# huangjh-pub/di-fusion

Hardware: AMD Instinct MI355X
Metric: frames/s integrate+decode+mesh, 640x480 synthetic stream (higher is better)
Workload: dtype f32

## Files before the change

### di_fusion_amd/csrc/kernels_extract.hip.h

```cpp
#pragma once

__device__ __forceinline__ void mark_confident_nbhd(const Geo& g, int lin, float ignore_th, const int64_t* __restrict__ indexer,
                                                    const float* __restrict__ obs, const GridMarks& marks) {
    const uint32_t* bits = marks.bits;
    int ix, iy, iz;
    unlinearize(g, lin, ix, iy, iz);
    int cand[7];
    cand[0] = lin;
    cand[1] = linearize(g, clampi(ix - 1, 0, g.nx - 1), iy, iz);
    cand[2] = linearize(g, clampi(ix + 1, 0, g.nx - 1), iy, iz);
    cand[3] = linearize(g, ix, clampi(iy - 1, 0, g.ny - 1), iz);
    cand[4] = linearize(g, ix, clampi(iy + 1, 0, g.ny - 1), iz);
    cand[5] = linearize(g, ix, iy, clampi(iz - 1, 0, g.nz - 1));
    cand[6] = linearize(g, ix, iy, clampi(iz + 1, 0, g.nz - 1));
    int64_t slot[7];
#pragma unroll
    for (int c = 0; c < 7; ++c) slot[c] = indexer[cand[c]];
    float w[7];
#pragma unroll
    for (int c = 0; c < 7; ++c) w[c] = slot[c] >= 0 ? obs[slot[c]] : ignore_th;
    uint32_t word[7];
#pragma unroll
    for (int c = 0; c < 7; ++c) word[c] = (w[c] > ignore_th) ? bits[cand[c] >> 5] : 0xFFFFFFFFu;
    uint32_t prev[7];
// ... 265 lines not shown
        if (R.live) {
            const int64_t p = A.list[row];
            float xn, yn, zn; int ix, iy, iz;
            voxel_of(A.geo, A.xyz[p * 3 + 0], A.xyz[p * 3 + 1], A.xyz[p * 3 + 2], xn, yn, zn, ix, iy, iz);
            R.px = (xn - (float)ix) - 0.5f; R.py = (yn - (float)iy) - 0.5f; R.pz = (zn - (float)iz) - 0.5f;
            lat_row = A.latent + A.indexer[linearize(A.geo, ix, iy, iz)] * L;
            R.out_idx = row;
        }
    }
#pragma unroll
    for (int t = 0; t < 16; ++t) {
        const int k = 2 * t + half;
        float v = 0.0f;
        if (R.live) {
            if (row32) v = row32[k];
            else if (k < L) v = lat_row[k];
            else v = (k == L) ? R.px : ((k == L + 1) ? R.py : R.pz);
        }
        xin[t] = v;
    }
    if constexpr (!DENSE) {
        if (A.mode == 2) {
            unsigned nf = 0;
#pragma unroll
            for (int t = 0; t < 16; ++t) nf |= ((__float_as_uint(xin[t]) & 0x7f800000u) == 0x7f800000u) ? 1u : 0u;
            nf |= (unsigned)__shfl_xor((int)nf, 32);
            R.bad = nf != 0;
        }
    }
    return R;
}

template <bool GRAD, bool DENSE = false>
__global__ void __launch_bounds__(GRAD ? 256 : 512, GRAD ? 1 : 2) k_decode(DecodeArgs A, const float* __restrict__ wblob) {
    extern __shared__ __attribute__((aligned(16))) float lds[];
    if (DENSE && A.zero_word && blockIdx.x == 0 && threadIdx.x == 0) *A.zero_word = 0;
    stage_weights(lds, wblob, DEC_LDS_FLOATS);
    const __amdgpu_buffer_rsrc_t wfwd = make_rsrc(wblob, DEC_FLOATS);
    const __amdgpu_buffer_rsrc_t wbwd = make_rsrc(GRAD ? A.wbwd : wblob, GRAD ? DECB_FLOATS : DEC_FLOATS);
    const int lane = lane_id(), half = lane >> 5, col = lane & 31;
    const int wave = (int)((threadIdx.x >> 6) * gridDim.x + blockIdx.x);
    const int nwaves = (int)(gridDim.x * (blockDim.x >> 6));
    const int res3 = A.lat.res * A.lat.res * A.lat.res;
    const int tiles_per_voxel = (res3 + 31) / 32;
    int64_t n_rows, n_tiles;
    if (A.mode == 0) {
        n_rows = (int64_t)(*A.n_ptr) * res3;
        n_tiles = (int64_t)(*A.n_ptr) * tiles_per_voxel;
    } else {
        n_rows = A.n_ptr ? (int64_t)(*A.n_ptr) : A.n_static;
        n_tiles = (n_rows + 31) / 32;
    }
    for (int64_t tile = wave; tile < n_tiles; tile += nwaves) {
        f16v xin;
        const DecodeRow R = decode_row_input<DENSE>(A, tile, col, half, res3, tiles_per_voxel, n_rows, xin);
        const bool live = R.live;
        const int64_t out_idx = R.out_idx;
        const float px = R.px, py = R.py, pz = R.pz;
        float sdf, sd;
        if (!GRAD && A.mode == 1 && A.fold_table) {
            const int b = live ? A.list[tile * 32 + col] / res3 : 0;
            decoder_tile_folded(lds, wfwd, FoldInitGlobal{A.fold_table + (int64_t)b * 256}, px, py, pz, lane, sdf, sd);
        } else if (GRAD) {
            float gx, gy, gz;
            decoder_tile_grad(lds, wfwd, wbwd, xin, lane, sdf, sd, gx, gy, gz);
            if (live && half == 1) {
                const float gs = R.bad ? __builtin_nanf("") : A.grad_scale;
                A.out_grad[out_idx * 3 + 0] = gx * gs;
                A.out_grad[out_idx * 3 + 1] = gy * gs;
                A.out_grad[out_idx * 3 + 2] = gz * gs;
            }
        } else {
            decoder_tile(lds, wfwd, xin, lane, sdf, sd);
        }
        if (live) {
            if (half == 0) A.out_sdf[out_idx] = R.bad ? __builtin_nanf("") : A.sign * sdf;
            else A.out_std[out_idx] = R.bad ? __builtin_nanf("") : sd;
        }
    }
}

template <bool DENSE = false>
__global__ void __launch_bounds__(512, 1) k_decode_x6(DecodeArgs A, const float* __restrict__ wblob, const float* __restrict__ wu) {
    extern __shared__ __attribute__((aligned(16))) float lds[];
    if (DENSE && A.zero_word && blockIdx.x == 0 && threadIdx.x == 0) *A.zero_word = 0;
    stage_weights(lds, wblob, X6_LDS_BYTES / 4);
    const __amdgpu_buffer_rsrc_t wfwd = make_rsrc(wblob, X6_BYTES / 4);
    const __amdgpu_buffer_rsrc_t wun = make_rsrc(wu, X6U_BYTES / 4);
    const int lane = lane_id(), half = lane >> 5, col = lane & 31;
    const int wave = (int)((threadIdx.x >> 6) * gridDim.x + blockIdx.x);
    const int nwaves = (int)(gridDim.x * (blockDim.x >> 6));
    const int res3 = A.lat.res * A.lat.res * A.lat.res;
    const int tiles_per_voxel = (res3 + 31) / 32;
    int64_t n_rows, n_tiles;
    if (A.mode == 0) {
        n_rows = (int64_t)(*A.n_ptr) * res3;
        n_tiles = (int64_t)(*A.n_ptr) * tiles_per_voxel;
    } else {
        n_rows = A.n_ptr ? (int64_t)(*A.n_ptr) : A.n_static;
        n_tiles = (n_rows + 31) / 32;
    }
    for (int64_t tile = wave; tile < n_tiles; tile += nwaves) {
        f16v xin;
        const DecodeRow R = decode_row_input<DENSE>(A, tile, col, half, res3, tiles_per_voxel, n_rows, xin);
        const bool live = R.live;
        const int64_t out_idx = R.out_idx;
        float sdf, sd;
        decoder_tile_x6(lds, wfwd, wun, xin, lane, sdf, sd);
        if (live) {
            if (half == 0) A.out_sdf[out_idx] = R.bad ? __builtin_nanf("") : A.sign * sdf;
            else A.out_std[out_idx] = R.bad ? __builtin_nanf("") : sd;
        }
    }
}

#ifndef GRAD_X6_THREADS
#define GRAD_X6_THREADS 256
#endif
template <int PF, bool DENSE = false>
__global__ void __launch_bounds__(GRAD_X6_THREADS, 1) k_decode_grad_x6(DecodeArgs A, const float* __restrict__ wblob, const float* __restrict__ wu,
                                                          const float* __restrict__ wb) {
    extern __shared__ __attribute__((aligned(16))) float lds[];
    if (DENSE && A.zero_word && blockIdx.x == 0 && threadIdx.x == 0) *A.zero_word = 0;
    stage_weights(lds, wblob, X6_LDS_BYTES / 4);
    const __amdgpu_buffer_rsrc_t wfwd = make_rsrc(wblob, X6_BYTES / 4);
    const __amdgpu_buffer_rsrc_t wun = make_rsrc(wu, X6U_BYTES / 4);
    const __amdgpu_buffer_rsrc_t wbw = make_rsrc(wb, X6B_BYTES / 4);
    const int lane = lane_id(), half = lane >> 5, col = lane & 31;
    const int wave = (int)((threadIdx.x >> 6) * gridDim.x + blockIdx.x);
    const int nwaves = (int)(gridDim.x * (blockDim.x >> 6));
    const int res3 = A.lat.res * A.lat.res * A.lat.res;
    const int64_t n_rows = A.n_ptr ? (int64_t)(*A.n_ptr) : A.n_static;
    const int64_t n_tiles = (n_rows + 31) / 32;
    for (int64_t tile = wave; tile < n_tiles; tile += nwaves) {
        f16v xin;
        const DecodeRow R = decode_row_input<DENSE>(A, tile, col, half, res3, 1, n_rows, xin);
        float sdf, sd, gx, gy, gz;
        decoder_tile_grad_x6<PF>(lds, wfwd, wun, wbw, xin, lane, sdf, sd, gx, gy, gz);
        if (R.live) {
            if (half == 0) A.out_sdf[R.out_idx] = R.bad ? __builtin_nanf("") : A.sign * sdf;
            else {
                const float gs = R.bad ? __builtin_nanf("") : A.grad_scale;
                A.out_std[R.out_idx] = R.bad ? __builtin_nanf("") : sd;
                A.out_grad[R.out_idx * 3 + 0] = gx * gs;
                A.out_grad[R.out_idx * 3 + 1] = gy * gs;
                A.out_grad[R.out_idx * 3 + 2] = gz * gs;
            }
        }
    }
}

template <int NS>
__device__ __forceinline__ void decode_refine_x6_body(const BatchN<DecodeArgs, NS>& B, int S, const float* __restrict__ wblob) {
    extern __shared__ __attribute__((aligned(16))) float lds[];
    const int lane = lane_id(), half = lane >> 5, col = lane & 31;
    const int wave = __builtin_amdgcn_readfirstlane((int)((threadIdx.x >> 6) * gridDim.x + blockIdx.x));
    const int nwaves = (int)(gridDim.x * (blockDim.x >> 6));
    const Lattice lat = B.s[0].lat;
    const float sign = B.s[0].sign;
    const int res3 = lat.res * lat.res * lat.res, r = lat.res;
    Ranges<NS, int64_t> rg;
    rg.pre[0] = 0;
#pragma unroll
    for (int j = 0; j < NS; ++j) {
        rg.cnt[j] = (j < S) ? (B.s[j].n_ptr ? (int64_t)(*B.s[j].n_ptr) : B.s[j].n_static) : 0;
        rg.pre[j + 1] = rg.pre[j] + (rg.cnt[j] + 31) / 32;
    }
    const int64_t n_tiles = rg.total();
    int sm_n; int64_t lt_n, rows_n;
    rg.locate(wave, sm_n, lt_n, rows_n);
    int e_next = (wave < n_tiles && lt_n * 32 + col < rows_n) ? B.s[sm_n].list[lt_n * 32 + col] : 0;
    __builtin_amdgcn_sched_barrier(0);
    stage_weights(lds, wblob, X6_LDS_BYTES / 4);
    const __amdgpu_buffer_rsrc_t wfwd = make_rsrc(wblob, X6_BYTES / 4);
    for (int64_t T = wave; T < n_tiles; T += nwaves) {
        const int sm = sm_n;
        const int64_t tile = lt_n, n_rows = rows_n;
        const DecodeArgs& A = B.s[sm];
        const int64_t row = tile * 32 + col;
        const bool live = row < n_rows;
        const int e = e_next;
        rg.locate(T + nwaves, sm_n, lt_n, rows_n);
        e_next = (T + nwaves < n_tiles && lt_n * 32 + col < rows_n) ? B.s[sm_n].list[lt_n * 32 + col] : 0;
        const int b = e / res3, sb = e - b * res3;
        const float px = lat.coord(sb / (r * r)), py = lat.coord((sb / r) % r), pz = lat.coord(sb % r);
        float sdf, sd;
        decoder_tile_folded_x6(lds, wfwd, FoldInitGlobal{A.fold_table + (int64_t)b * 256}, px, py, pz, lane, sdf, sd);
        if (live) {
            if (half == 0) A.out_sdf[e] = sign * sdf;
            else A.out_std[e] = sd;
        }
    }
}

__global__ void __launch_bounds__(512, 1) k_decode_refine_x6(DecodeArgs A, const float* __restrict__ wblob) {
    const BatchN<DecodeArgs, 1> B{{A}};
    decode_refine_x6_body<1>(B, 1, wblob);
}
__global__ void __launch_bounds__(512, 1) k_decode_refine_x6_batch(Batch<DecodeArgs> B, int S, const float* __restrict__ wblob) {
    decode_refine_x6_body<DIF_MAX_STREAMS>(B, S, wblob);
}

__device__ __forceinline__ void tri_axis(int j, int l, float scale, int& i0, int& i1, float& w0, float& w1) {
    float src = scale * (float)j;
    i0 = min((int)src, l - 1);
    i1 = i0 + ((i0 < l - 1) ? 1 : 0);
    w1 = fminf(fmaxf(src - (float)i0, 0.0f), 1.0f);
    w0 = 1.0f - w1;
}

__device__ __forceinline__ float tri_sample(const float* __restrict__ low, int l, int x0, int x1, int y0, int y1, int z0, int z1,
                                            float wx0, float wx1, float wy0, float wy1, float wz0, float wz1) {
    float v00 = fmaf(low[(x0 * l + y0) * l + z0], wz0, low[(x0 * l + y0) * l + z1] * wz1);
    float v01 = fmaf(low[(x0 * l + y1) * l + z0], wz0, low[(x0 * l + y1) * l + z1] * wz1);
    float v10 = fmaf(low[(x1 * l + y0) * l + z0], wz0, low[(x1 * l + y0) * l + z1] * wz1);
    float v11 = fmaf(low[(x1 * l + y1) * l + z0], wz0, low[(x1 * l + y1) * l + z1] * wz1);
    float v0 = fmaf(v00, wy0, v01 * wy1);
    float v1 = fmaf(v10, wy0, v11 * wy1);
    return fmaf(v0, wx0, v1 * wx1);
}

__global__ void __launch_bounds__(DIF_BLOCK) k_upsample_mark(const float* __restrict__ low_sdf, const float* __restrict__ low_std, int l, int R,
                                                           float* __restrict__ cube_sdf, float* __restrict__ cube_std,
                                                           int32_t* __restrict__ refine_list, int* __restrict__ counters) {
    __shared__ int smem[8];
    __shared__ int s_base;
    const int B = counters[DIF_C_B];
    const int R2 = R * R, R3 = R2 * R, l3 = l * l * l;
    const int64_t n_rows = (int64_t)B * R2;
    const float scale = (float)(l - 1) / (float)(R - 1);
    const int64_t stride = (int64_t)gridDim.x * blockDim.x;
    const int64_t n_pad = (n_rows + DIF_BLOCK - 1) / DIF_BLOCK * DIF_BLOCK;
    for (int64_t row = (int64_t)blockIdx.x * blockDim.x + threadIdx.x; row < n_pad; row += stride) {
        unsigned sel = 0;
        int64_t e0 = 0;
        if (row < n_rows) {
            const int b = (int)(row / R2), jxy = (int)(row - (int64_t)b * R2);
            const int jx = jxy / R, jy = jxy % R;
            int x0, x1, y0, y1; float wx0, wx1, wy0, wy1;
            tri_axis(jx, l, scale, x0, x1, wx0, wx1);
            tri_axis(jy, l, scale, y0, y1, wy0, wy1);
            const float* ls = low_sdf + (int64_t)b * l3;
            const float* ld = low_std + (int64_t)b * l3;
            e0 = (int64_t)b * R3 + (int64_t)jxy * R;
            NO_PACKED_F32
            for (int jz = 0; jz < R; ++jz) {
                int z0, z1; float wz0, wz1;
                tri_axis(jz, l, scale, z0, z1, wz0, wz1);
                float sv = tri_sample(ls, l, x0, x1, y0, y1, z0, z1, wx0, wx1, wy0, wy1, wz0, wz1);
                float dv = tri_sample(ld, l, x0, x1, y0, y1, z0, z1, wx0, wx1, wy0, wy1, wz0, wz1);
                cube_sdf[e0 + jz] = -sv;
                cube_std[e0 + jz] = dv;
                if (fabsf(sv) < 0.05f) sel |= 1u << jz;
            }
        }
        int total;
        int ex = block_excl_scan(__popc(sel), smem, total);
        if (total > 0) {
            if (threadIdx.x == 0) s_base = atomicAdd(counters + DIF_C_VH, total);
            __syncthreads();
            int o = s_base + ex;
            while (sel) {
                int jz = __ffs((int)sel) - 1;
                sel &= sel - 1;
                refine_list[o++] = (int32_t)(e0 + jz);
            }
        }
        __syncthreads();
    }
}

struct VoxelDecodeArgs {
    const int32_t* occ_slot;
    const float* latent;
    Lattice low;
    int R;
    float* cube_sdf;
    float* cube_std;
    int32_t* refine_list;
    int* counters;
    const float* fold_w;
    float* fold_table;
};

#define VD_MAX_L3 64
#define VD_MAX_R2 64
#define VD_WAVE_LDS_FLOATS (2 * VD_MAX_L3 + 2 * 256)

#ifdef DIF_TRACE
__device__ unsigned long long g_vd_trace[2048 * 8];
#define VD_STAMP(slot) do { if (lane_id() == 0) g_vd_trace[((threadIdx.x >> 6) * gridDim.x + blockIdx.x) * 8 + (slot)] = wall_clock64(); } while (0)
#else
#define VD_STAMP(slot) do { } while (0)
#endif

template <bool X6, int NS>
__device__ __forceinline__ void decode_voxels_body(const BatchN<VoxelDecodeArgs, NS>& AB, int S, const float* __restrict__ wblob) {
    extern __shared__ __attribute__((aligned(16))) float lds[];
    VD_STAMP(0);
    constexpr int LDS_W = X6 ? X6_LDS_BYTES / 4 : ((DEC_LDS_FLOATS + 3) & ~3);
#if defined(DIF_VD_CUT) && DIF_VD_CUT == 0
    return;
#endif
    stage_weights(lds, wblob, X6 ? X6_LDS_BYTES / 4 : DEC_LDS_FLOATS);
    VD_STAMP(1);
#if defined(DIF_VD_CUT) && DIF_VD_CUT == 1
    return;
#endif
    const __amdgpu_buffer_rsrc_t wfwd = make_rsrc(wblob, X6 ? X6_BYTES / 4 : DEC_FLOATS);
    const int lane = lane_id(), half = lane >> 5, col = lane & 31, wid = threadIdx.x >> 6;
    const int pair = wid >> 1, tsel = wid & 1;
    float* w_low_sdf = lds + LDS_W + pair * VD_WAVE_LDS_FLOATS;
    float* w_low_std = w_low_sdf + VD_MAX_L3;
    float* w_fold = w_low_std + VD_MAX_L3 + tsel * 256;
    const Lattice low = AB.s[0].low;
    const float* const fold_w = AB.s[0].fold_w;
    const int l = low.res, R = AB.s[0].R, l3 = l * l * l, R2 = R * R, R3 = R2 * R;
    const float scale = (float)(l - 1) / (float)(R - 1);
    int pre[NS + 1];
    pre[0] = 0;
#pragma unroll
    for (int j = 0; j < NS; ++j) pre[j + 1] = pre[j] + ((j < S) ? AB.s[j].counters[DIF_C_B] : 0);
    const int B = pre[NS];
    const int pairs_per_block = (int)(blockDim.x >> 7), n_pairs = (int)gridDim.x * pairs_per_block;
    const int first = __builtin_amdgcn_readfirstlane(pair * (int)gridDim.x + (int)blockIdx.x);
    __shared__ int s_tot[8], s_map[8], s_base[NS];
    const int rounds = (B + n_pairs - 1) / n_pairs;
    for (int round = 0; round < rounds; ++round) {
        const int bg = first + round * n_pairs;
        int sm = 0, b = bg;
#pragma unroll
        for (int j = 1; j < NS; ++j)
            if (bg >= pre[j]) { sm = j; b = bg - pre[j]; }
        const VoxelDecodeArgs& A = AB.s[sm];
        unsigned sel = 0;
        const int jz0 = tsel * (R >> 1), jz1 = jz0 + (R >> 1);
        const int64_t e0 = (int64_t)b * R3 + (int64_t)lane * R;
        if (bg < B && tsel * 32 < l3) {
            const float* lat_row = A.latent + (int64_t)A.occ_slot[b] * L;
            const int s = tsel * 32 + col;
            const float px = low.coord(s / (l * l)), py = low.coord((s / l) % l), pz = low.coord(s % l);
            float sdf = 0.0f, sd = 0.0f;
            if (X6 || fold_w) {
                if constexpr (X6) decoder_fold_consts_x6(lds, fold_w, lat_row, w_fold, lane);
                else decoder_fold_consts(lds, fold_w, lat_row, w_fold, lane);
                __builtin_amdgcn_wave_barrier();
                __builtin_amdgcn_s_waitcnt(0xc07f);
                if (tsel == 0) {
                    float* rec = A.fold_table + (int64_t)b * 256;
                    for (int p = lane; p < 256; p += 64) rec[p] = w_fold[p];
                }
                VD_STAMP(6);
#if defined(DIF_VD_CUT) && DIF_VD_CUT == 2
                sdf = w_fold[lane]; sd = w_fold[lane + 64];
#else
                if constexpr (X6) decoder_tile_folded_x6(lds, wfwd, FoldInitLds{w_fold}, px, py, pz, lane, sdf, sd);
                else decoder_tile_folded(lds, wfwd, FoldInitLds{w_fold}, px, py, pz, lane, sdf, sd);
#endif
            } else if constexpr (!X6) {
                f16v xin;
#pragma unroll
                for (int t = 0; t < 16; ++t) {
                    const int k = 2 * t + half;
                    xin[t] = (k < L) ? lat_row[k] : 0.0f;
                }
                if (half) { xin[14] = px; xin[15] = pz; } else { xin[15] = py; }
                decoder_tile(lds, wfwd, xin, lane, sdf, sd);
            }
            if (s < l3) {
                if (half == 0) w_low_sdf[s] = sdf;
                else w_low_std[s] = sd;
            }
        }
        __syncthreads();
        VD_STAMP(2);
        if (bg < B && lane < R2) {
            const int jx = lane / R, jy = lane % R;
            int x0, x1, y0, y1; float wx0, wx1, wy0, wy1;
            tri_axis(jx, l, scale, x0, x1, wx0, wx1);
            tri_axis(jy, l, scale, y0, y1, wy0, wy1);
            float* const cube_sdf = A.cube_sdf;
            float* const cube_std = A.cube_std;
            for (int jz = jz0; jz < jz1; ++jz) {
                int z0, z1; float wz0, wz1;
                tri_axis(jz, l, scale, z0, z1, wz0, wz1);
                float sv = tri_sample(w_low_sdf, l, x0, x1, y0, y1, z0, z1, wx0, wx1, wy0, wy1, wz0, wz1);
                float dv = tri_sample(w_low_std, l, x0, x1, y0, y1, z0, z1, wx0, wx1, wy0, wy1, wz0, wz1);
                cube_sdf[e0 + jz] = -sv;
                cube_std[e0 + jz] = dv;
                if (fabsf(sv) < 0.05f) sel |= 1u << jz;
            }
        }
        VD_STAMP(3);
        const int c = __popc(sel);
        const int incl = wave_incl_scan(c);
        const int total = __shfl(incl, 63);
        if (lane == 0) { s_tot[wid] = total; if (NS > 1) s_map[wid] = sm; }
        __syncthreads();
        if (NS == 1) {
            if (threadIdx.x == 0) {
                int sum = 0;
                for (int w = 0; w < (int)(blockDim.x >> 6); ++w) sum += s_tot[w];
                s_base[0] = sum ? atomicAdd(A.counters + DIF_C_VH, sum) : 0;
            }
        } else if ((int)threadIdx.x < S) {
            const int j = (int)threadIdx.x;
            int sum = 0;
            for (int w = 0; w < (int)(blockDim.x >> 6); ++w) sum += (s_map[w] == j) ? s_tot[w] : 0;
            s_base[j] = sum ? atomicAdd(AB.s[j].counters + DIF_C_VH, sum) : 0;
        }
        __syncthreads();
        if (total > 0) {
            int o = s_base[NS == 1 ? 0 : sm] + incl - c;
            for (int w = 0; w < wid; ++w) o += (NS == 1 || s_map[w] == sm) ? s_tot[w] : 0;
            int32_t* const refine_list = A.refine_list;
            while (sel) {
                const int jz = __ffs((int)sel) - 1;
                sel &= sel - 1;
                refine_list[o++] = (int32_t)(e0 + jz);
            }
        }
        __syncthreads();
        VD_STAMP(4);
    }
    VD_STAMP(5);
}

template <bool X6>
__global__ void __launch_bounds__(512, X6 ? 1 : 2) k_decode_voxels(VoxelDecodeArgs A, const float* __restrict__ wblob) {
    const BatchN<VoxelDecodeArgs, 1> B{{A}};
    decode_voxels_body<X6, 1>(B, 1, wblob);
}
template <bool X6>
__global__ void __launch_bounds__(512, X6 ? 1 : 2) k_decode_voxels_batch(Batch<VoxelDecodeArgs> B, int S, const float* __restrict__ wblob) {
    decode_voxels_body<X6, DIF_MAX_STREAMS>(B, S, wblob);
}
```

### di_fusion_amd/csrc/mlp.hip.h

```cpp
#pragma once
#include "common.hip.h"

namespace dif {

typedef float f16v __attribute__((ext_vector_type(16)));
typedef float f4v __attribute__((ext_vector_type(4)));

__device__ __forceinline__ f16v mfma32(float a, float b, f16v c) { return __builtin_amdgcn_mfma_f32_32x32x2f32(a, b, c, 0, 0, 0); }

__device__ __forceinline__ f16v load_bias16(const float* b, int half) {
    const f4v* p = reinterpret_cast<const f4v*>(b + half * 16);
    f4v b0 = p[0], b1 = p[1], b2 = p[2], b3 = p[3];
    f16v r;
    r[0] = b0.x; r[1] = b0.y; r[2] = b0.z; r[3] = b0.w;
    r[4] = b1.x; r[5] = b1.y; r[6] = b1.z; r[7] = b1.w;
    r[8] = b2.x; r[9] = b2.y; r[10] = b2.z; r[11] = b2.w;
    r[12] = b3.x; r[13] = b3.y; r[14] = b3.z; r[15] = b3.w;
    return r;
}

__device__ __forceinline__ float relu1(float x) { return __int_as_float(max(__float_as_int(x), 0)); }
__device__ __forceinline__ f16v relu16(f16v v) {
#pragma unroll
    for (int i = 0; i < 16; ++i) v[i] = relu1(v[i]);
    return v;
}

typedef unsigned int u4v __attribute__((ext_vector_type(4)));

struct LdsA {
    const f4v* p;
    __device__ __forceinline__ f4v load(int t, int lane) const { return p[t * 64 + lane]; }
};

struct BufA {
    __amdgpu_buffer_rsrc_t rsrc;
    int base;
    __device__ __forceinline__ f4v load(int t, int lane) const {
        u4v v = __builtin_amdgcn_raw_buffer_load_b128(rsrc, lane * 16, base + t * 1024, 0);
        return __builtin_bit_cast(f4v, v);
    }
};

__device__ __forceinline__ __amdgpu_buffer_rsrc_t make_rsrc(const float* p, int n_floats) {
    return __builtin_amdgcn_make_buffer_rsrc((void*)p, 0, n_floats * 4, 0x00020000);
}

template <int NB, class ASRC>
__device__ __forceinline__ f16v block_mm_src(const ASRC& A, const f16v (&hin)[NB], f16v acc, int lane) {
    f4v a = A.load(0, lane);
#pragma unroll
    for (int kb = 0; kb < NB; ++kb) {
#pragma unroll
        for (int g = 0; g < 4; ++g) {
            const int t = kb * 4 + g;
            f4v an = a;
            if (t + 1 < NB * 4) an = A.load(t + 1, lane);
            acc = mfma32(a.x, hin[kb][4 * g + 0], acc);
            acc = mfma32(a.y, hin[kb][4 * g + 1], acc);
            acc = mfma32(a.z, hin[kb][4 * g + 2], acc);
            acc = mfma32(a.w, hin[kb][4 * g + 3], acc);
            a = an;
            __builtin_amdgcn_sched_barrier(0);
        }
    }
    return acc;
}

template <int NMB, int NB, int PF>
__device__ __forceinline__ void stream_mm(const BufA& A, const f16v (&hin)[NB], f16v (&acc)[NMB], int lane) {
    constexpr int NU = NMB * NB * 4;
    f4v ring[PF];
#pragma unroll
    for (int i = 0; i < PF; ++i)
        if (i < NU) ring[i] = A.load(i, lane);
#pragma unroll
    for (int mb = 0; mb < NMB; ++mb) {
#pragma unroll
        for (int kb = 0; kb < NB; ++kb) {
#pragma unroll
            for (int g = 0; g < 4; ++g) {
                const int u = (mb * NB + kb) * 4 + g;
                const f4v a = ring[u % PF];
                if (u + PF < NU) ring[u % PF] = A.load(u + PF, lane);
                acc[mb] = mfma32(a.x, hin[kb][4 * g + 0], acc[mb]);
                acc[mb] = mfma32(a.y, hin[kb][4 * g + 1], acc[mb]);
                acc[mb] = mfma32(a.z, hin[kb][4 * g + 2], acc[mb]);
                acc[mb] = mfma32(a.w, hin[kb][4 * g + 3], acc[mb]);
                __builtin_amdgcn_sched_barrier(0);
            }
        }
    }
}

template <int NB>
__device__ __forceinline__ f16v block_mm(const f4v* __restrict__ A, const f16v (&hin)[NB], f16v acc, int lane) {
    return block_mm_src<NB>(LdsA{A}, hin, acc, lane);
}

#define ENC_A0 0
#define ENC_B0 256
#define ENC_A1 288
#define ENC_B1 2336
#define ENC_A2 2400
#define ENC_B2 18784
#define ENC_A3 19040
#define ENC_B3 27232
#define ENC_FLOATS 27264

__device__ __forceinline__ f16v encoder_tile(const float* __restrict__ W , float x0, float x1, float x2, int lane) {
    const int half = lane >> 5;
    f16v h0[1];
    {
        f16v acc = load_bias16(W + ENC_B0, half);
        f4v a = reinterpret_cast<const f4v*>(W + ENC_A0)[lane];
        acc = mfma32(a.x, x0, acc);
        acc = mfma32(a.y, x1, acc);
        acc = mfma32(a.z, x2, acc);
        h0[0] = relu16(acc);
    }
    f16v h1[2];
#pragma unroll
    for (int mb = 0; mb < 2; ++mb) {
        f16v acc = load_bias16(W + ENC_B1 + mb * 32, half);
        acc = block_mm<1>(reinterpret_cast<const f4v*>(W + ENC_A1) + (mb * 4) * 64, h0, acc, lane);
        h1[mb] = relu16(acc);
    }
    f16v out = load_bias16(W + ENC_B3, half);
#pragma unroll
    for (int mb = 0; mb < 8; ++mb) {
        f16v acc = load_bias16(W + ENC_B2 + mb * 32, half);
        acc = block_mm<2>(reinterpret_cast<const f4v*>(W + ENC_A2) + (mb * 8) * 64, h1, acc, lane);
        f16v h2[1];
        h2[0] = relu16(acc);
        out = block_mm<1>(reinterpret_cast<const f4v*>(W + ENC_A3) + (mb * 4) * 64, h2, out, lane);
    }
    return out;
}

#define DEC_A0 0
#define DEC_B0 4096
#define DEC_A1 4224
#define DEC_B1 20608
#define DEC_A2 20736
#define DEC_B2 33024
#define DEC_B3 33120
#define DEC_HW 33248
#define DEC_HU 33376
#define DEC_HB 33504
#define DEC_LDS_FLOATS 33508
#define DEC_A3 33508
#define DEC_FLOATS 49892

__device__ __forceinline__ void decoder_tile(const float* __restrict__ W , __amdgpu_buffer_rsrc_t Wg ,
                                             const f16v& xin, int lane, float& sdf, float& stdv) {
    const int half = lane >> 5;
    f16v hx[1];
    hx[0] = xin;
    f16v h0[4];
#pragma unroll
    for (int mb = 0; mb < 4; ++mb) {
        f16v acc = load_bias16(W + DEC_B0 + mb * 32, half);
        acc = block_mm<1>(reinterpret_cast<const f4v*>(W + DEC_A0) + (mb * 4) * 64, hx, acc, lane);
        h0[mb] = relu16(acc);
    }
    f16v h1[4];
#pragma unroll
    for (int mb = 0; mb < 4; ++mb) {
        f16v acc = load_bias16(W + DEC_B1 + mb * 32, half);
        acc = block_mm<4>(reinterpret_cast<const f4v*>(W + DEC_A1) + (mb * 16) * 64, h0, acc, lane);
        h1[mb] = relu16(acc);
    }
    f16v h2x[4];
#pragma unroll
    for (int mb = 0; mb < 3; ++mb) {
        f16v acc = load_bias16(W + DEC_B2 + mb * 32, half);
        acc = block_mm<4>(reinterpret_cast<const f4v*>(W + DEC_A2) + (mb * 16) * 64, h1, acc, lane);
        h2x[mb] = relu16(acc);
    }
    h2x[3] = xin;
    int off3 = DEC_A3 * 4;
    asm volatile("" : "+s"(off3) : : "memory");
    float ps = 0.0f, pu = 0.0f;
#pragma unroll
    for (int mb = 0; mb < 4; ++mb) {
        f16v acc = load_bias16(W + DEC_B3 + mb * 32, half);
        acc = block_mm_src<4>(BufA{Wg, off3 + mb * 16 * 1024}, h2x, acc, lane);
        acc = relu16(acc);
        f16v ws = load_bias16(W + DEC_HW + mb * 32, half);
        f16v wu = load_bias16(W + DEC_HU + mb * 32, half);
#pragma unroll
        for (int r = 0; r < 16; ++r) {
            ps = fmaf(acc[r], ws[r], ps);
            pu = fmaf(acc[r], wu[r], pu);
        }
    }
    ps += __shfl_xor(ps, 32);
    pu += __shfl_xor(pu, 32);
    ps += W[DEC_HB + 0];
    pu += W[DEC_HB + 1];
    sdf = tanhf(ps);
    float sp = (pu > 20.0f) ? pu : log1pf(expf(pu));
    stdv = 0.05f + 0.5f * sp;
}

#define DECF_FLOATS (2 * 29 * 128)

template <int B0, int B3, int UNROLL>
__device__ __forceinline__ void decoder_fold_consts_at(const float* __restrict__ W , const float* __restrict__ fold ,
                                                       const float* __restrict__ lat_row, float* __restrict__ c, int lane) {
    float a0 = W[B0 + lane], a1 = W[B0 + lane + 64], a2 = W[B3 + lane], a3 = W[B3 + lane + 64];
    const f4v* wk = reinterpret_cast<const f4v*>(fold) + lane;
#pragma unroll UNROLL
    for (int k = 0; k < 29; ++k) {
        const float zk = lat_row[k];
        const f4v wv = wk[k * 64];
        a0 = fmaf(wv.x, zk, a0);
        a1 = fmaf(wv.y, zk, a1);
        a2 = fmaf(wv.z, zk, a2);
        a3 = fmaf(wv.w, zk, a3);
    }
    c[lane] = a0;
    c[lane + 64] = a1;
    c[128 + lane] = a2;
    c[128 + lane + 64] = a3;
}
__device__ __forceinline__ void decoder_fold_consts(const float* __restrict__ W, const float* __restrict__ fold, const float* __restrict__ lat_row,
                                                    float* __restrict__ c, int lane) {
    decoder_fold_consts_at<DEC_B0, DEC_B3, 8>(W, fold, lat_row, c, lane);
}

struct FoldInitLds {
    const float* c;
    __device__ __forceinline__ f16v load(int layer, int mb, int half) const { return load_bias16(c + layer * 128 + mb * 32, half); }
};
struct FoldInitGlobal {
    const float* rec;
    __device__ __forceinline__ f16v load(int layer, int mb, int half) const { return load_bias16(rec + layer * 128 + mb * 32, half); }
};

template <class INIT>
__device__ __forceinline__ void decoder_tile_folded(const float* __restrict__ W , __amdgpu_buffer_rsrc_t Wg , const INIT& init,
                                                    float px, float py, float pz, int lane, float& sdf, float& stdv) {
    const int half = lane >> 5;
    const float b14 = half ? px : 0.0f;
    const float b15 = half ? pz : py;
    f16v h0[4];
#pragma unroll
    for (int mb = 0; mb < 4; ++mb) {
        f16v acc = init.load(0, mb, half);
        const f4v a = reinterpret_cast<const f4v*>(W + DEC_A0)[(mb * 4 + 3) * 64 + lane];
        acc = mfma32(a.z, b14, acc);
        acc = mfma32(a.w, b15, acc);
        h0[mb] = relu16(acc);
        __builtin_amdgcn_sched_barrier(0);
    }
    f16v h1[4];
#pragma unroll
    for (int mb = 0; mb < 4; ++mb) {
        f16v acc = load_bias16(W + DEC_B1 + mb * 32, half);
        acc = block_mm<4>(reinterpret_cast<const f4v*>(W + DEC_A1) + (mb * 16) * 64, h0, acc, lane);
        h1[mb] = relu16(acc);
    }
    f16v h2[3];
#pragma unroll
    for (int mb = 0; mb < 3; ++mb) {
        f16v acc = load_bias16(W + DEC_B2 + mb * 32, half);
        acc = block_mm<4>(reinterpret_cast<const f4v*>(W + DEC_A2) + (mb * 16) * 64, h1, acc, lane);
        h2[mb] = relu16(acc);
    }
    int off3 = DEC_A3 * 4;
    asm volatile("" : "+s"(off3) : : "memory");
    float ps = 0.0f, pu = 0.0f;
#pragma unroll
    for (int mb = 0; mb < 4; ++mb) {
        f16v acc = init.load(1, mb, half);
        const BufA src{Wg, off3 + mb * 16 * 1024};
        const f4v ax = src.load(15, lane);
        acc = block_mm_src<3>(src, h2, acc, lane);
        acc = mfma32(ax.z, b14, acc);
        acc = mfma32(ax.w, b15, acc);
        __builtin_amdgcn_sched_barrier(0);
        acc = relu16(acc);
        f16v ws = load_bias16(W + DEC_HW + mb * 32, half);
        f16v wu = load_bias16(W + DEC_HU + mb * 32, half);
#pragma unroll
        for (int r = 0; r < 16; ++r) {
            ps = fmaf(acc[r], ws[r], ps);
            pu = fmaf(acc[r], wu[r], pu);
        }
    }
    ps += __shfl_xor(ps, 32);
    pu += __shfl_xor(pu, 32);
    ps += W[DEC_HB + 0];
    pu += W[DEC_HB + 1];
    sdf = tanhf(ps);
    float sp = (pu > 20.0f) ? pu : log1pf(expf(pu));
    stdv = 0.05f + 0.5f * sp;
}

typedef __bf16 bf8v __attribute__((ext_vector_type(8)));
struct Tri { u4v q0, q1, q2; };

__device__ __forceinline__ f16v mfb(u4v a, u4v b, f16v c) {
    return __builtin_amdgcn_mfma_f32_32x32x16_bf16(__builtin_bit_cast(bf8v, a), __builtin_bit_cast(bf8v, b), c, 0, 0, 0);
}
typedef __bf16 bf2v __attribute__((ext_vector_type(2)));
typedef float f2v __attribute__((ext_vector_type(2)));
__device__ __forceinline__ unsigned cvt_pk_bf16(float lo, float hi) {
    return __builtin_bit_cast(unsigned, __builtin_convertvector(f2v{lo, hi}, bf2v));
}
__device__ __forceinline__ void split_pair(float a, float b, unsigned& p0, unsigned& p1, unsigned& p2) {
    p0 = cvt_pk_bf16(a, b);
    const float ra = a - __uint_as_float(p0 << 16), rb = b - __uint_as_float(p0 & 0xffff0000u);
    p1 = cvt_pk_bf16(ra, rb);
    const float sa = ra - __uint_as_float(p1 << 16), sb = rb - __uint_as_float(p1 & 0xffff0000u);
    p2 = cvt_pk_bf16(sa, sb);
}
__device__ __forceinline__ void split_pair_into(const f16v& h, int s, int p, Tri& t) {
    unsigned p0, p1, p2;
    split_pair(h[8 * s + 2 * p], h[8 * s + 2 * p + 1], p0, p1, p2);
    t.q0[p] = p0; t.q1[p] = p1; t.q2[p] = p2;
}

struct LdsX6 {
    const u4v* p;
    __device__ __forceinline__ Tri load(int t, int lane) const { const u4v* q = p + t * 192 + lane; return Tri{q[0], q[64], q[128]}; }
};
struct BufX6 {
    __amdgpu_buffer_rsrc_t rsrc;
    int base;
    __device__ __forceinline__ Tri load(int t, int lane) const {
        const int o = base + t * 3072;
        return Tri{__builtin_amdgcn_raw_buffer_load_b128(rsrc, lane * 16, o, 0), __builtin_amdgcn_raw_buffer_load_b128(rsrc, lane * 16 + 1024, o, 0),
                   __builtin_amdgcn_raw_buffer_load_b128(rsrc, lane * 16 + 2048, o, 0)};
    }
};

__device__ __forceinline__ f16v step_x6(const Tri& a, const Tri& x, f16v c) {
    c = mfb(a.q2, x.q0, c);
    c = mfb(a.q1, x.q1, c);
    c = mfb(a.q0, x.q2, c);
    c = mfb(a.q1, x.q0, c);
    c = mfb(a.q0, x.q1, c);
    c = mfb(a.q0, x.q0, c);
    return c;
}

template <int KB0, int KB1, int NMO, int PF, class SRC>
__device__ __forceinline__ void layer_x6(const SRC& A, const f16v* hin, f16v* acc, int lane) {
    constexpr int NS = (KB1 - KB0) * 2 * NMO;
    Tri ring[PF];
#pragma unroll
    for (int i = 0; i < PF; ++i)
        if (i < NS) ring[i] = A.load(i, lane);
    Tri x[2], xn[2];
#pragma unroll
    for (int i = 0; i < 8; ++i) split_pair_into(hin[KB0], i >> 2, i & 3, x[i >> 2]);
#pragma unroll
    for (int kb = KB0; kb < KB1; ++kb) {
#pragma unroll
        for (int s = 0; s < 2; ++s) {
#pragma unroll
            for (int mo = 0; mo < NMO; ++mo) {
                const int u = s * NMO + mo;
                const int t = (kb - KB0) * 2 * NMO + u;
                const Tri a = ring[t % PF];
                if (t + PF < NS) ring[t % PF] = A.load(t + PF, lane);
                if (kb + 1 < KB1) {
                    constexpr int per = (8 + 2 * NMO - 1) / (2 * NMO);
#pragma unroll
                    for (int i = u * per; i < (u + 1) * per && i < 8; ++i) split_pair_into(hin[kb + 1], i >> 2, i & 3, xn[i >> 2]);
                }
                acc[mo] = step_x6(a, x[s], acc[mo]);
                __builtin_amdgcn_sched_barrier(0);
            }
        }
        if (kb + 1 < KB1) { x[0] = xn[0]; x[1] = xn[1]; }
    }
}

#ifndef X6_PF_LDS
#define X6_PF_LDS 2
#endif
#define X6_A0C 0
#define X6_B0 1024
#define X6_B1 1152
#define X6_B2 1280
#define X6_B3 1376
#define X6_HW 1504
#define X6_HU 1632
#define X6_HB 1760
#define X6_A3C 1764
#define X6_AUX_FLOATS 2788
#define X6_L1 (X6_AUX_FLOATS * 4)
#define X6_L2 (X6_L1 + 98304)
#define X6_LDS_BYTES (X6_L2 + 36864)
#define X6_L3 (X6_L2 + 73728)
#define X6_BYTES (X6_L3 + 73728)

__device__ __forceinline__ void decoder_fold_consts_x6(const float* __restrict__ aux , const float* __restrict__ fold ,
                                                       const float* __restrict__ lat_row, float* __restrict__ c, int lane) {
    decoder_fold_consts_at<X6_B0, X6_B3, 15>(aux, fold, lat_row, c, lane);
}

template <class INIT>
__device__ __forceinline__ void decoder_tile_folded_x6(const float* __restrict__ W , __amdgpu_buffer_rsrc_t Wg, const INIT& init,
                                                       float px, float py, float pz, int lane, float& sdf, float& stdv) {
    const int half = lane >> 5;
    const float b14 = half ? px : 0.0f;
    const float b15 = half ? pz : py;
    const char* Wb = reinterpret_cast<const char*>(W);
    f16v h0[4];
#pragma unroll
    for (int mb = 0; mb < 4; ++mb) {
        f16v acc = init.load(0, mb, half);
        const f4v a = reinterpret_cast<const f4v*>(W + X6_A0C)[mb * 64 + lane];
        acc = mfma32(a.z, b14, acc);
        acc = mfma32(a.w, b15, acc);
        h0[mb] = relu16(acc);
    }
    f16v h1[4];
#pragma unroll
    for (int mb = 0; mb < 4; ++mb) h1[mb] = load_bias16(W + X6_B1 + mb * 32, half);
    layer_x6<0, 4, 4, X6_PF_LDS>(LdsX6{reinterpret_cast<const u4v*>(Wb + X6_L1)}, h0, h1, lane);
#pragma unroll
    for (int mb = 0; mb < 4; ++mb) h1[mb] = relu16(h1[mb]);
    f16v h2[3];
#pragma unroll
    for (int mb = 0; mb < 3; ++mb) h2[mb] = load_bias16(W + X6_B2 + mb * 32, half);
    int goff = X6_L2 + 36864;
    asm volatile("" : "+s"(goff) : : "memory");
    layer_x6<0, 2, 3, X6_PF_LDS>(LdsX6{reinterpret_cast<const u4v*>(Wb + X6_L2)}, h1, h2, lane);
    layer_x6<2, 4, 3, 3>(BufX6{Wg, goff}, h1, h2, lane);
#pragma unroll
    for (int mb = 0; mb < 3; ++mb) h2[mb] = relu16(h2[mb]);
    f16v h3[4];
#pragma unroll
    for (int mb = 0; mb < 4; ++mb) h3[mb] = init.load(1, mb, half);
    layer_x6<0, 3, 4, 3>(BufX6{Wg, goff + 36864}, h2, h3, lane);
    float ps = 0.0f, pu = 0.0f;
#pragma unroll
    for (int mb = 0; mb < 4; ++mb) {
        f16v acc = h3[mb];
        const f4v ax = reinterpret_cast<const f4v*>(W + X6_A3C)[mb * 64 + lane];
        acc = mfma32(ax.z, b14, acc);
        acc = mfma32(ax.w, b15, acc);
        acc = relu16(acc);
        f16v ws = load_bias16(W + X6_HW + mb * 32, half);
        f16v wu = load_bias16(W + X6_HU + mb * 32, half);
#pragma unroll
        for (int r = 0; r < 16; ++r) {
            ps = fmaf(acc[r], ws[r], ps);
            pu = fmaf(acc[r], wu[r], pu);
        }
    }
    ps += __shfl_xor(ps, 32);
    pu += __shfl_xor(pu, 32);
    ps += W[X6_HB + 0];
    pu += W[X6_HB + 1];
    sdf = tanhf(ps);
    float sp = (pu > 20.0f) ? pu : log1pf(expf(pu));
    stdv = 0.05f + 0.5f * sp;
}

#define X6U_L0 0
#define X6U_L3X 24576
#define X6U_BYTES 49152
__device__ __forceinline__ void decoder_tile_x6(const float* __restrict__ W , __amdgpu_buffer_rsrc_t Wg, __amdgpu_buffer_rsrc_t Wu,
                                                const f16v& xin, int lane, float& sdf, float& stdv) {
    const int half = lane >> 5;
    const char* Wb = reinterpret_cast<const char*>(W);
    int uoff = X6U_L0, goff = X6_L2 + 36864;
    asm volatile("" : "+s"(uoff), "+s"(goff) : : "memory");
    f16v hx[1];
    hx[0] = xin;
    f16v h0[4];
#pragma unroll
    for (int mb = 0; mb < 4; ++mb) h0[mb] = load_bias16(W + X6_B0 + mb * 32, half);
    layer_x6<0, 1, 4, 3>(BufX6{Wu, uoff}, hx, h0, lane);
#pragma unroll
    for (int mb = 0; mb < 4; ++mb) h0[mb] = relu16(h0[mb]);
    f16v h1[4];
#pragma unroll
    for (int mb = 0; mb < 4; ++mb) h1[mb] = load_bias16(W + X6_B1 + mb * 32, half);
    layer_x6<0, 4, 4, X6_PF_LDS>(LdsX6{reinterpret_cast<const u4v*>(Wb + X6_L1)}, h0, h1, lane);
#pragma unroll
    for (int mb = 0; mb < 4; ++mb) h1[mb] = relu16(h1[mb]);
    f16v h2[3];
#pragma unroll
    for (int mb = 0; mb < 3; ++mb) h2[mb] = load_bias16(W + X6_B2 + mb * 32, half);
    layer_x6<0, 2, 3, X6_PF_LDS>(LdsX6{reinterpret_cast<const u4v*>(Wb + X6_L2)}, h1, h2, lane);
    layer_x6<2, 4, 3, 3>(BufX6{Wg, goff}, h1, h2, lane);
#pragma unroll
    for (int mb = 0; mb < 3; ++mb) h2[mb] = relu16(h2[mb]);
    f16v h3[4];
#pragma unroll
    for (int mb = 0; mb < 4; ++mb) h3[mb] = load_bias16(W + X6_B3 + mb * 32, half);
    layer_x6<0, 3, 4, 3>(BufX6{Wg, goff + 36864}, h2, h3, lane);
    layer_x6<0, 1, 4, 3>(BufX6{Wu, uoff + X6U_L3X}, hx, h3, lane);
    float ps = 0.0f, pu = 0.0f;
#pragma unroll
    for (int mb = 0; mb < 4; ++mb) {
        const f16v acc = relu16(h3[mb]);
        f16v ws = load_bias16(W + X6_HW + mb * 32, half);
        f16v wu = load_bias16(W + X6_HU + mb * 32, half);
#pragma unroll
        for (int r = 0; r < 16; ++r) {
            ps = fmaf(acc[r], ws[r], ps);
            pu = fmaf(acc[r], wu[r], pu);
        }
    }
    ps += __shfl_xor(ps, 32);
    pu += __shfl_xor(pu, 32);
    ps += W[X6_HB + 0];
    pu += W[X6_HB + 1];
    sdf = tanhf(ps);
    float sp = (pu > 20.0f) ? pu : log1pf(expf(pu));
    stdv = 0.05f + 0.5f * sp;
}

#define E6_A0 0
#define E6_B0 256
#define E6_B1 288
#define E6_B2 352
#define E6_B3 608
#define E6_AUX_FLOATS 640
#define E6_L1 (E6_AUX_FLOATS * 4)
#define E6_L23 (E6_L1 + 12288)
#define E6_BYTES (E6_L23 + 147456)

__device__ __forceinline__ f16v encoder_tile_x6(const float* __restrict__ W , float x0, float x1, float x2, int lane) {
    const int half = lane >> 5;
    const char* Wb = reinterpret_cast<const char*>(W);
    f16v h0[1];
    {
        f16v acc = load_bias16(W + E6_B0, half);
        f4v a = reinterpret_cast<const f4v*>(W + E6_A0)[lane];
        acc = mfma32(a.x, x0, acc);
        acc = mfma32(a.y, x1, acc);
        acc = mfma32(a.z, x2, acc);
        h0[0] = relu16(acc);
    }
    f16v h1[2];
    h1[0] = load_bias16(W + E6_B1, half);
    h1[1] = load_bias16(W + E6_B1 + 32, half);
    layer_x6<0, 1, 2, 1>(LdsX6{reinterpret_cast<const u4v*>(Wb + E6_L1)}, h0, h1, lane);
    h1[0] = relu16(h1[0]);
    h1[1] = relu16(h1[1]);
    Tri xs[4];
#pragma unroll
    for (int i = 0; i < 16; ++i) split_pair_into(h1[i >> 3], (i >> 2) & 1, i & 3, xs[i >> 2]);
    const LdsX6 A{reinterpret_cast<const u4v*>(Wb + E6_L23)};
    int t = 0;
    Tri a = A.load(0, lane), an;
    f16v cur = load_bias16(W + E6_B2, half);
#pragma unroll
    for (int u = 0; u < 4; ++u) {
        an = A.load(t + 1, lane);
        cur = step_x6(a, xs[u], cur);
        a = an; ++t;
        __builtin_amdgcn_sched_barrier(0);
    }
    f16v out = load_bias16(W + E6_B3, half);
#pragma unroll
    for (int mb = 0; mb < 8; ++mb) {
        const f16v h = relu16(cur);
        Tri hs[2];
        if (mb + 1 < 8) {
            cur = load_bias16(W + E6_B2 + (mb + 1) * 32, half);
#pragma unroll
            for (int u = 0; u < 4; ++u) {
                an = A.load(t + 1, lane);
                split_pair_into(h, u >> 1, (2 * u) & 3, hs[u >> 1]);
                split_pair_into(h, u >> 1, (2 * u + 1) & 3, hs[u >> 1]);
                cur = step_x6(a, xs[u], cur);
                a = an; ++t;
                __builtin_amdgcn_sched_barrier(0);
            }
        } else {
#pragma unroll
            for (int i = 0; i < 8; ++i) split_pair_into(h, i >> 2, i & 3, hs[i >> 2]);
        }
#pragma unroll
        for (int s = 0; s < 2; ++s) {
            an = a;
            if (t + 1 < 48) an = A.load(t + 1, lane);
            out = step_x6(a, hs[s], out);
            a = an; ++t;
            __builtin_amdgcn_sched_barrier(0);
        }
    }
    return out;
}

#define DECB_T3 0
#define DECB_T2 16384
#define DECB_T1 28672
#define DECB_T0 45056
#define DECB_FLOATS 49152

__device__ __forceinline__ f16v relu16_mask(f16v v, unsigned& mask) {
    unsigned m = 0;
#pragma unroll
    for (int i = 0; i < 16; ++i) {
        m |= (v[i] > 0.0f) ? (1u << i) : 0u;
        v[i] = fmaxf(v[i], 0.0f);
    }
    mask = m;
    return v;
}

__device__ __forceinline__ f16v apply_mask16(f16v v, unsigned mask) {
#pragma unroll
    for (int i = 0; i < 16; ++i) v[i] = ((mask >> i) & 1u) ? v[i] : 0.0f;
    return v;
}

__device__ __forceinline__ f16v zero16() {
    f16v z;
#pragma unroll
    for (int i = 0; i < 16; ++i) z[i] = 0.0f;
    return z;
}

#define GRAD_PF 8
__device__ __forceinline__ void decoder_tile_grad(const float* __restrict__ W , __amdgpu_buffer_rsrc_t Wg ,
                                                  __amdgpu_buffer_rsrc_t Wb , const f16v& xin, int lane,
                                                  float& sdf, float& stdv, float& gx, float& gy, float& gz) {
    const int half = lane >> 5;
    unsigned m0[4], m1[4], m2[3], m3[4];
    f16v hx[1];
    hx[0] = xin;
    f16v h0[4];
#pragma unroll
    for (int mb = 0; mb < 4; ++mb) {
        f16v acc = load_bias16(W + DEC_B0 + mb * 32, half);
        acc = block_mm<1>(reinterpret_cast<const f4v*>(W + DEC_A0) + (mb * 4) * 64, hx, acc, lane);
        h0[mb] = relu16_mask(acc, m0[mb]);
    }
    f16v h1[4];
#pragma unroll
    for (int mb = 0; mb < 4; ++mb) {
        f16v acc = load_bias16(W + DEC_B1 + mb * 32, half);
        acc = block_mm<4>(reinterpret_cast<const f4v*>(W + DEC_A1) + (mb * 16) * 64, h0, acc, lane);
        h1[mb] = relu16_mask(acc, m1[mb]);
    }
    f16v h2x[4];
#pragma unroll
    for (int mb = 0; mb < 3; ++mb) {
        f16v acc = load_bias16(W + DEC_B2 + mb * 32, half);
        acc = block_mm<4>(reinterpret_cast<const f4v*>(W + DEC_A2) + (mb * 16) * 64, h1, acc, lane);
        h2x[mb] = relu16_mask(acc, m2[mb]);
    }
    h2x[3] = xin;
    int off3 = DEC_A3 * 4, offb = 0;
    asm volatile("" : "+s"(off3), "+s"(offb) : : "memory");
    float ps = 0.0f, pu = 0.0f;
    f16v g3[4];
    f16v h3[4];
#pragma unroll
    for (int mb = 0; mb < 4; ++mb) h3[mb] = load_bias16(W + DEC_B3 + mb * 32, half);
    stream_mm<4, 4, GRAD_PF>(BufA{Wg, off3}, h2x, h3, lane);
#pragma unroll
    for (int mb = 0; mb < 4; ++mb) {
        f16v acc = relu16_mask(h3[mb], m3[mb]);
        f16v ws = load_bias16(W + DEC_HW + mb * 32, half);
        f16v wu = load_bias16(W + DEC_HU + mb * 32, half);
#pragma unroll
        for (int r = 0; r < 16; ++r) {
            ps = fmaf(acc[r], ws[r], ps);
            pu = fmaf(acc[r], wu[r], pu);
        }
        g3[mb] = apply_mask16(ws, m3[mb]);
    }
    ps += __shfl_xor(ps, 32);
    pu += __shfl_xor(pu, 32);
    ps += W[DEC_HB + 0];
    pu += W[DEC_HB + 1];
    sdf = tanhf(ps);
    float sp = (pu > 20.0f) ? pu : log1pf(expf(pu));
    stdv = 0.05f + 0.5f * sp;
    f16v t3[4];
#pragma unroll
    for (int mb = 0; mb < 4; ++mb) t3[mb] = zero16();
    stream_mm<4, 4, GRAD_PF>(BufA{Wb, offb + DECB_T3 * 4}, g3, t3, lane);
    f16v g2[3];
#pragma unroll
    for (int mb = 0; mb < 3; ++mb) g2[mb] = apply_mask16(t3[mb], m2[mb]);
    f16v g1[4];
#pragma unroll
    for (int mb = 0; mb < 4; ++mb) g1[mb] = zero16();
    stream_mm<4, 3, GRAD_PF>(BufA{Wb, offb + DECB_T2 * 4}, g2, g1, lane);
#pragma unroll
    for (int mb = 0; mb < 4; ++mb) g1[mb] = apply_mask16(g1[mb], m1[mb]);
    f16v g0[4];
#pragma unroll
    for (int mb = 0; mb < 4; ++mb) g0[mb] = zero16();
    stream_mm<4, 4, GRAD_PF>(BufA{Wb, offb + DECB_T1 * 4}, g1, g0, lane);
#pragma unroll
    for (int mb = 0; mb < 4; ++mb) g0[mb] = apply_mask16(g0[mb], m0[mb]);
    f16v gx1[1];
    gx1[0] = t3[3];
    stream_mm<1, 4, GRAD_PF>(BufA{Wb, offb + DECB_T0 * 4}, g0, gx1, lane);
    const f16v gxv = gx1[0];
// ... 294 lines not shown
```

Measured before the change: 9895.

## Prefetch next latent row, defer refine-list writes, batch fold-weight loads

The voxel decode loop now fetches the next round's occupancy slot and latent vector into a register (one latent element per lane) while the current round is still computing, and reads latent values with readlane instead of global loads. The refine-list atomic reservation and list writes are deferred by one round using double-buffered shared counters, which removes one __syncthreads per round. The fold-constant loop issues its weight loads in batches fenced by scheduling barriers, so the loads can be in flight together. This adds register pressure and more complex control flow, and it relies on the latent length being at most the 64-lane wave width.

Measured after the change: 8974. -9.3%, worse.

```diff
diff --git a/di_fusion_amd/csrc/kernels_extract.hip.h b/di_fusion_amd/csrc/kernels_extract.hip.h
--- a/di_fusion_amd/csrc/kernels_extract.hip.h
+++ b/di_fusion_amd/csrc/kernels_extract.hip.h
@@ -591,17 +591,8 @@
 #if defined(DIF_VD_CUT) && DIF_VD_CUT == 0
     return;
 #endif
-    stage_weights(lds, wblob, X6 ? X6_LDS_BYTES / 4 : DEC_LDS_FLOATS);
-    VD_STAMP(1);
-#if defined(DIF_VD_CUT) && DIF_VD_CUT == 1
-    return;
-#endif
-    const __amdgpu_buffer_rsrc_t wfwd = make_rsrc(wblob, X6 ? X6_BYTES / 4 : DEC_FLOATS);
     const int lane = lane_id(), half = lane >> 5, col = lane & 31, wid = threadIdx.x >> 6;
     const int pair = wid >> 1, tsel = wid & 1;
-    float* w_low_sdf = lds + LDS_W + pair * VD_WAVE_LDS_FLOATS;
-    float* w_low_std = w_low_sdf + VD_MAX_L3;
-    float* w_fold = w_low_std + VD_MAX_L3 + tsel * 256;
     const Lattice low = AB.s[0].low;
     const float* const fold_w = AB.s[0].fold_w;
     const int l = low.res, R = AB.s[0].R, l3 = l * l * l, R2 = R * R, R3 = R2 * R;
@@ -613,26 +604,88 @@
     const int B = pre[NS];
     const int pairs_per_block = (int)(blockDim.x >> 7), n_pairs = (int)gridDim.x * pairs_per_block;
     const int first = __builtin_amdgcn_readfirstlane(pair * (int)gridDim.x + (int)blockIdx.x);
-    __shared__ int s_tot[8], s_map[8], s_base[NS];
+    const bool has_tile = tsel * 32 < l3;
+    auto locate = [&](int bg, int& sm, int& b) {
+        sm = 0; b = bg;
+#pragma unroll
+        for (int j = 1; j < NS; ++j)
+            if (bg >= pre[j]) { sm = j; b = bg - pre[j]; }
+    };
+    stage_weights(lds, wblob, X6 ? X6_LDS_BYTES / 4 : DEC_LDS_FLOATS);
+    VD_STAMP(1);
+#if defined(DIF_VD_CUT) && DIF_VD_CUT == 1
+    return;
+#endif
+    int sm_n, b_n, slot_n = 0;
+    float z_n = 0.0f;
+    locate(first, sm_n, b_n);
+    if (first < B && has_tile) {
+        slot_n = AB.s[sm_n].occ_slot[b_n];
+        if (lane < L) z_n = AB.s[sm_n].latent[(int64_t)slot_n * L + lane];
+    }
+    const __amdgpu_buffer_rsrc_t wfwd = make_rsrc(wblob, X6 ? X6_BYTES / 4 : DEC_FLOATS);
+    float* w_low_sdf = lds + LDS_W + pair * VD_WAVE_LDS_FLOATS;
+    float* w_low_std = w_low_sdf + VD_MAX_L3;
+    float* w_fold = w_low_std + VD_MAX_L3 + tsel * 256;
+    __shared__ int s_tot[2][8], s_map[2][8], s_base[2][NS];
+    const int jz0 = tsel * (R >> 1), jz1 = jz0 + (R >> 1);
+    auto in_vgpr = [](int* p) { int zero_v = 0; asm volatile("" : "+v"(zero_v)); return p + zero_v; };
+    int pend = 0;
+    auto reserve = [&](int q) {
+        if (NS == 1) {
+            if (threadIdx.x == 0) {
+                int sum = 0;
+                for (int w = 0; w < (int)(blockDim.x >> 6); ++w) sum += s_tot[q][w];
+                pend = sum ? atomicAdd(in_vgpr(AB.s[0].counters + DIF_C_VH), sum) : 0;
+            }
+        } else if ((int)threadIdx.x < S) {
+            const int j = (int)threadIdx.x;
+            int sum = 0;
+            for (int w = 0; w < (int)(blockDim.x >> 6); ++w) sum += (s_map[q][w] == j) ? s_tot[q][w] : 0;
+            pend = sum ? atomicAdd(in_vgpr(AB.s[j].counters + DIF_C_VH), sum) : 0;
+        }
+    };
+    auto publish = [&](int q) {
+        if (NS == 1) { if (threadIdx.x == 0) s_base[q][0] = pend; }
+        else if ((int)threadIdx.x < S) s_base[q][threadIdx.x] = pend;
+    };
+    unsigned p_sel = 0;
+    int p_excl = 0, p_sm = 0, p_b = 0;
+    auto write_list = [&](int q) {
+        if (p_sel) {
+            int o = s_base[q][NS == 1 ? 0 : p_sm] + p_excl;
+            for (int w = 0; w < wid; ++w) o += (NS == 1 || s_map[q][w] == p_sm) ? s_tot[q][w] : 0;
+            int32_t* const refine_list = AB.s[p_sm].refine_list;
+            const int64_t e0 = (int64_t)p_b * R3 + (int64_t)lane * R;
+            while (p_sel) {
+                const int jz = __ffs((int)p_sel) - 1;
+                p_sel &= p_sel - 1;
+                refine_list[o++] = (int32_t)(e0 + jz);
+            }
+        }
+    };
     const int rounds = (B + n_pairs - 1) / n_pairs;
     for (int round = 0; round < rounds; ++round) {
+        const int cur = round & 1, prv = cur ^ 1;
         const int bg = first + round * n_pairs;
-        int sm = 0, b = bg;
-#pragma unroll
-        for (int j = 1; j < NS; ++j)
-            if (bg >= pre[j]) { sm = j; b = bg - pre[j]; }
+        const int sm = sm_n, b = b_n;
+        const LatentLanes lat_row{z_n};
         const VoxelDecodeArgs& A = AB.s[sm];
-        unsigned sel = 0;
-        const int jz0 = tsel * (R >> 1), jz1 = jz0 + (R >> 1);
-        const int64_t e0 = (int64_t)b * R3 + (int64_t)lane * R;
-        if (bg < B && tsel * 32 < l3) {
-            const float* lat_row = A.latent + (int64_t)A.occ_slot[b] * L;
-            const int s = tsel * 32 + col;
-            const float px = low.coord(s / (l * l)), py = low.coord((s / l) % l), pz = low.coord(s % l);
+        const bool tile = bg < B && has_tile;
+        const bool tile_n = bg + n_pairs < B && has_tile;
+        locate(bg + n_pairs, sm_n, b_n);
+        if (tile_n) slot_n = AB.s[sm_n].occ_slot[b_n];
+        const int s = tsel * 32 + col;
+        const float px = low.coord(s / (l * l)), py = low.coord((s / l) % l), pz = low.coord(s % l);
+        const bool folded = X6 || fold_w;
+        int zero_s = 0;
+        asm volatile("" : "+s"(zero_s));
+        const float* const fold_r = fold_w + zero_s;
+        if (tile) {
             float sdf = 0.0f, sd = 0.0f;
-            if (X6 || fold_w) {
-                if constexpr (X6) decoder_fold_consts_x6(lds, fold_w, lat_row, w_fold, lane);
-                else decoder_fold_consts(lds, fold_w, lat_row, w_fold, lane);
+            if (folded) {
+                if constexpr (X6) decoder_fold_consts_x6(lds, fold_r, lat_row, w_fold, lane);
+                else decoder_fold_consts(lds, fold_r, lat_row, w_fold, lane);
                 __builtin_amdgcn_wave_barrier();
                 __builtin_amdgcn_s_waitcnt(0xc07f);
                 if (tsel == 0) {
@@ -640,6 +693,8 @@
                     for (int p = lane; p < 256; p += 64) rec[p] = w_fold[p];
                 }
                 VD_STAMP(6);
+            }
+            if (folded) {
 #if defined(DIF_VD_CUT) && DIF_VD_CUT == 2
                 sdf = w_fold[lane]; sd = w_fold[lane + 64];
 #else
@@ -650,8 +705,8 @@
                 f16v xin;
 #pragma unroll
                 for (int t = 0; t < 16; ++t) {
-                    const int k = 2 * t + half;
-                    xin[t] = (k < L) ? lat_row[k] : 0.0f;
+                    const float ze = lat_row[2 * t], zo = (2 * t + 1 < L) ? lat_row[2 * t + 1] : 0.0f;
+                    xin[t] = (2 * t < L) ? (half ? zo : ze) : 0.0f;
                 }
                 if (half) { xin[14] = px; xin[15] = pz; } else { xin[15] = py; }
                 decoder_tile(lds, wfwd, xin, lane, sdf, sd);
@@ -661,9 +716,14 @@
                 else w_low_std[s] = sd;
             }
         }
+        if (tile_n && lane < L) z_n = AB.s[sm_n].latent[(int64_t)__builtin_amdgcn_readfirstlane(slot_n) * L + lane];
+        if (round > 0) publish(prv);
         __syncthreads();
         VD_STAMP(2);
+        if (round > 0) write_list(prv);
+        unsigned sel = 0;
         if (bg < B && lane < R2) {
+            const int64_t e0 = (int64_t)b * R3 + (int64_t)lane * R;
             const int jx = lane / R, jy = lane % R;
             int x0, x1, y0, y1; float wx0, wx1, wy0, wy1;
             tri_axis(jx, l, scale, x0, x1, wx0, wx1);
@@ -683,34 +743,17 @@
         VD_STAMP(3);
         const int c = __popc(sel);
         const int incl = wave_incl_scan(c);
-        const int total = __shfl(incl, 63);
-        if (lane == 0) { s_tot[wid] = total; if (NS > 1) s_map[wid] = sm; }
+        if (lane == 63) { s_tot[cur][wid] = incl; if (NS > 1) s_map[cur][wid] = sm; }
+        p_sel = sel; p_excl = incl - c; p_sm = sm; p_b = b;
         __syncthreads();
-        if (NS == 1) {
-            if (threadIdx.x == 0) {
-                int sum = 0;
-                for (int w = 0; w < (int)(blockDim.x >> 6); ++w) sum += s_tot[w];
-                s_base[0] = sum ? atomicAdd(A.counters + DIF_C_VH, sum) : 0;
-            }
-        } else if ((int)threadIdx.x < S) {
-            const int j = (int)threadIdx.x;
-            int sum = 0;
-            for (int w = 0; w < (int)(blockDim.x >> 6); ++w) sum += (s_map[w] == j) ? s_tot[w] : 0;
-            s_base[j] = sum ? atomicAdd(AB.s[j].counters + DIF_C_VH, sum) : 0;
-        }
+        reserve(cur);
+        VD_STAMP(4);
+    }
+    if (rounds > 0) {
+        const int q = (rounds - 1) & 1;
+        publish(q);
         __syncthreads();
-        if (total > 0) {
-            int o = s_base[NS == 1 ? 0 : sm] + incl - c;
-            for (int w = 0; w < wid; ++w) o += (NS == 1 || s_map[w] == sm) ? s_tot[w] : 0;
-            int32_t* const refine_list = A.refine_list;
-            while (sel) {
-                const int jz = __ffs((int)sel) - 1;
-                sel &= sel - 1;
-                refine_list[o++] = (int32_t)(e0 + jz);
-            }
-        }
-        __syncthreads();
-        VD_STAMP(4);
+        write_list(q);
     }
     VD_STAMP(5);
 }
diff --git a/di_fusion_amd/csrc/mlp.hip.h b/di_fusion_amd/csrc/mlp.hip.h
--- a/di_fusion_amd/csrc/mlp.hip.h
+++ b/di_fusion_amd/csrc/mlp.hip.h
@@ -206,26 +206,40 @@
 
 #define DECF_FLOATS (2 * 29 * 128)
 
-template <int B0, int B3, int UNROLL>
+struct LatentLanes {
+    float zlane;
+    __device__ __forceinline__ float operator[](int k) const { return __int_as_float(__builtin_amdgcn_readlane(__float_as_int(zlane), k)); }
+};
+
+template <int B0, int B3, int BATCH>
 __device__ __forceinline__ void decoder_fold_consts_at(const float* __restrict__ W , const float* __restrict__ fold ,
-                                                       const float* __restrict__ lat_row, float* __restrict__ c, int lane) {
+                                                       const LatentLanes lat_row, float* __restrict__ c, int lane) {
     float a0 = W[B0 + lane], a1 = W[B0 + lane + 64], a2 = W[B3 + lane], a3 = W[B3 + lane + 64];
     const f4v* wk = reinterpret_cast<const f4v*>(fold) + lane;
-#pragma unroll UNROLL
-    for (int k = 0; k < 29; ++k) {
-        const float zk = lat_row[k];
-        const f4v wv = wk[k * 64];
-        a0 = fmaf(wv.x, zk, a0);
-        a1 = fmaf(wv.y, zk, a1);
-        a2 = fmaf(wv.z, zk, a2);
-        a3 = fmaf(wv.w, zk, a3);
+#pragma unroll
+    for (int k0 = 0; k0 < 29; k0 += BATCH) {
+        f4v wv[BATCH];
+#pragma unroll
+        for (int i = 0; i < BATCH; ++i)
+            if (k0 + i < 29) wv[i] = wk[(k0 + i) * 64];
+        __builtin_amdgcn_sched_barrier(0);
+#pragma unroll
+        for (int i = 0; i < BATCH; ++i)
+            if (k0 + i < 29) {
+                const float zk = lat_row[k0 + i];
+                a0 = fmaf(wv[i].x, zk, a0);
+                a1 = fmaf(wv[i].y, zk, a1);
+                a2 = fmaf(wv[i].z, zk, a2);
+                a3 = fmaf(wv[i].w, zk, a3);
+            }
+        __builtin_amdgcn_sched_barrier(0);
     }
     c[lane] = a0;
     c[lane + 64] = a1;
     c[128 + lane] = a2;
     c[128 + lane + 64] = a3;
 }
-__device__ __forceinline__ void decoder_fold_consts(const float* __restrict__ W, const float* __restrict__ fold, const float* __restrict__ lat_row,
+__device__ __forceinline__ void decoder_fold_consts(const float* __restrict__ W, const float* __restrict__ fold, const LatentLanes lat_row,
                                                     float* __restrict__ c, int lane) {
     decoder_fold_consts_at<DEC_B0, DEC_B3, 8>(W, fold, lat_row, c, lane);
 }
@@ -400,7 +414,7 @@
 #define X6_BYTES (X6_L3 + 73728)
 
 __device__ __forceinline__ void decoder_fold_consts_x6(const float* __restrict__ aux , const float* __restrict__ fold ,
-                                                       const float* __restrict__ lat_row, float* __restrict__ c, int lane) {
+                                                       const LatentLanes lat_row, float* __restrict__ c, int lane) {
     decoder_fold_consts_at<X6_B0, X6_B3, 15>(aux, fold, lat_row, c, lane);
 }
 
```
